# ntnu-yjyjames/nano-vectordb

Measured on AMD Instinct MI355X. Metric: QPS + effective HBM GB/s, flat-scan top-10 d=768, higher is better.
Workload: dtype f16

## Files before the change

nano-vectordb_amd/csrc/kernels_exact.h:

```cpp
#pragma once
#include <hip/hip_runtime.h>

#include "nvdb_common.h"

namespace nvdbhip {

struct Cand { float score; uint32_t row; };

constexpr int DT_F32 = 1, DT_F16 = 2, DT_I8 = 3;
constexpr float NEG_INF = -__builtin_huge_valf();

__device__ __forceinline__ bool better(float s1, uint32_t i1, float s2, uint32_t i2) {
  return (s1 > s2) || (s1 == s2 && i1 < i2);
}
__device__ __forceinline__ float half_bits_to_float(uint32_t h16) {
  return static_cast<float>(__builtin_bit_cast(_Float16, static_cast<unsigned short>(h16)));
}
__device__ __forceinline__ float readlane_f(float v, int l) {
  return __builtin_bit_cast(float, __builtin_amdgcn_readlane(__builtin_bit_cast(int, v), l));
}
__device__ __forceinline__ uint32_t readlane_u(uint32_t v, int l) {
  return static_cast<uint32_t>(__builtin_amdgcn_readlane(static_cast<int>(v), l));
}
__device__ __forceinline__ float hsum8(const float (&a)[8]) {
// ... 200 lines not shown
  if (wave != 0) return;
#pragma unroll
  for (int g = 0; g < QG; ++g) {
    for (int w = 1; w < 4; ++w) {
      const uint32_t c = lds_cnt[w][g];
      for (uint32_t j = 0; j < c; ++j) {
        const float cs = lds_s[w][g][j];
        const uint32_t cid = lds_id[w][g][j];
        if (wtk_accepts(tk[g], k, cs, cid)) wtk_insert(tk[g], k, cs, cid, lane);
      }
    }
    const uint32_t qi = qbase + g;
    const bool own = qi >= qg0 && qi < nq;
    if (own && tk[g].cnt > 0) {
      uint32_t slot0 = 0;
      if (lane == 0) slot0 = atomicAdd(&cnt[qi], tk[g].cnt);
      slot0 = readlane_u(slot0, 0);
      if (static_cast<uint32_t>(lane) < tk[g].cnt) {
        const uint32_t slot = slot0 + lane;
        if (slot < cap) cand[static_cast<uint64_t>(qi) * cap + slot] = Cand{tk[g].s, tk[g].id};
        else overflow[qi] = 1u;
      }
    }
  }
}

__device__ __forceinline__ void fold_sticky_words(uint32_t* any_overflow) {
  const uint32_t viol = __hip_atomic_load(any_overflow - 6, __ATOMIC_RELAXED, __HIP_MEMORY_SCOPE_AGENT);
  const uint32_t logovf = __hip_atomic_load(any_overflow - 5, __ATOMIC_RELAXED, __HIP_MEMORY_SCOPE_AGENT);
  if (viol) atomicAdd(any_overflow + 7, viol);
  if (logovf) atomicOr(any_overflow + 8, 1u);
}

__device__ __forceinline__ void select_body(
    const uint32_t q, const uint32_t tid, const uint32_t nth, Cand* e,
    Cand* __restrict__ cand, uint32_t* __restrict__ cnt, uint32_t cap, uint32_t k, const float* __restrict__ slack,
    float* __restrict__ thr, uint32_t* __restrict__ overflow, int mode, uint64_t row_base,
    unsigned long long* __restrict__ out_ids, float* __restrict__ out_scores, uint32_t out_k, uint32_t* __restrict__ any_overflow,
    float* __restrict__ xcdw, bool fold_sticky) {
  __shared__ uint32_t s_keep;
  if (xcdw != nullptr && q == 0 && tid == 0) {
    float sp[8], mean = 0.f;
    bool all = true;
#pragma unroll
    for (int x = 0; x < 8; ++x) {
      const float us = xcdw[8 + x], tiles = xcdw[16 + x];
      all = all && us > 0.f && tiles > 0.f;
      sp[x] = tiles / fmaxf(us, 1e-3f);
      mean += sp[x] * 0.125f;
    }
    if (all) {
      float w[8], wsum = 0.f;
#pragma unroll
      for (int x = 0; x < 8; ++x) {
        w[x] = fminf(fmaxf(0.5f * xcdw[x] + 0.5f * sp[x] / mean, 0.9f), 1.1f);
        wsum += w[x];
      }
#pragma unroll
      for (int x = 0; x < 8; ++x) xcdw[x] = w[x] * (8.f / wsum);
    }
#pragma unroll
    for (int x = 8; x < 24; ++x) xcdw[x] = 0.f;
  }
  uint32_t m = (mode == 2) ? out_k : cnt[q];
  if (m > cap) { if (tid == 0) overflow[q] = 1u; m = cap; }
  if ((mode & 1) && tid == 0) {
    if (overflow[q]) { atomicOr(any_overflow, 1u); if (mode == 1) atomicOr(any_overflow + 6, 1u); }
    if (mode == 1 && fold_sticky) fold_sticky_words(any_overflow);
  }
  Cand* mine = cand + static_cast<uint64_t>(q) * cap;
  if (m <= 512) {
    __shared__ float s_kth;
    if (tid == 0) { s_keep = 0; s_kth = NEG_INF; }
    for (uint32_t i = tid; i < m; i += nth) e[i] = mine[i];
    __syncthreads();
    Cand my[2];
    uint32_t rk[2] = {0xFFFFFFFFu, 0xFFFFFFFFu};
#pragma unroll
    for (int u = 0; u < 2; ++u) {
      const uint32_t i = tid + u * nth;
      if (i < m) {
        my[u] = e[i];
        uint32_t r = 0;
        uint32_t j = 0;
        for (; j + 8 <= m; j += 8) {
          Cand o[8];
#pragma unroll
          for (int v = 0; v < 8; ++v) o[v] = e[j + v];
#pragma unroll
          for (int v = 0; v < 8; ++v) r += better(o[v].score, o[v].row, my[u].score, my[u].row) ? 1u : 0u;
        }
        for (; j < m; ++j) { const Cand o = e[j]; r += better(o.score, o.row, my[u].score, my[u].row) ? 1u : 0u; }
        rk[u] = r;
        if (r == k - 1) s_kth = my[u].score;
      }
    }
    __syncthreads();
    if (mode & 1) {
      const uint32_t c = m < k ? m : k;
#pragma unroll
      for (int u = 0; u < 2; ++u)
        if (rk[u] < c) { out_ids[static_cast<uint64_t>(q) * out_k + rk[u]] = row_base + my[u].row; out_scores[static_cast<uint64_t>(q) * out_k + rk[u]] = my[u].score; }
      for (uint32_t j = c + tid; j < out_k; j += nth) { out_ids[static_cast<uint64_t>(q) * out_k + j] = ~0ull; out_scores[static_cast<uint64_t>(q) * out_k + j] = NEG_INF; }
      return;
    }
    const float sl = slack ? slack[q] : 0.f;
    const float t = fmaxf(s_kth - sl, thr[q]);
    uint32_t local = 0;
#pragma unroll
    for (int u = 0; u < 2; ++u) if (rk[u] != 0xFFFFFFFFu) local += (sl > 0.f ? (my[u].score >= t) : (rk[u] < k)) ? 1u : 0u;
    if (local) atomicAdd(&s_keep, local);
    __syncthreads();
    const uint32_t keep = s_keep;
#pragma unroll
    for (int u = 0; u < 2; ++u) if (rk[u] < keep) mine[rk[u]] = my[u];
    if (tid == 0) { cnt[q] = (mode == 2) ? 0u : keep; thr[q] = t; }
    return;
  }
  uint32_t M2 = 1;
  while (M2 < m) M2 <<= 1;
  for (uint32_t i = tid; i < M2; i += nth) e[i] = (i < m) ? mine[i] : Cand{NEG_INF, 0xFFFFFFFFu};
  __syncthreads();
  for (uint32_t size = 2; size <= M2; size <<= 1) {
    for (uint32_t stride = size >> 1; stride > 0; stride >>= 1) {
      for (uint32_t i = tid; i < (M2 >> 1); i += nth) {
        const uint32_t a = 2 * i - (i & (stride - 1));
        const uint32_t b = a + stride;
        const bool desc = ((a & size) == 0);
        const Cand ea = e[a], eb = e[b];
        const bool b_better = better(eb.score, eb.row, ea.score, ea.row);
        if (b_better == desc) { e[a] = eb; e[b] = ea; }
      }
      __syncthreads();
    }
  }
  if (mode & 1) {
    const uint32_t c = m < k ? m : k;
    for (uint32_t j = tid; j < out_k; j += nth) {
      const bool have = j < c;
      out_ids[static_cast<uint64_t>(q) * out_k + j] = have ? (row_base + e[j].row) : ~0ull;
      out_scores[static_cast<uint64_t>(q) * out_k + j] = have ? e[j].score : NEG_INF;
    }
    return;
  }
  const float kth = (m >= k) ? e[k - 1].score : NEG_INF;
  const float sl = slack ? slack[q] : 0.f;
  const float t = fmaxf(kth - sl, thr[q]);
  if (tid == 0) s_keep = 0;
  __syncthreads();
  uint32_t local = 0;
  if (sl > 0.f) { for (uint32_t i = tid; i < m; i += nth) local += (e[i].score >= t) ? 1u : 0u; }
  else { for (uint32_t i = tid; i < m; i += nth) local += (i < k) ? 1u : 0u; }
  if (local) atomicAdd(&s_keep, local);
  __syncthreads();
  const uint32_t keep = s_keep;
  for (uint32_t i = tid; i < keep; i += nth) mine[i] = e[i];
  if (tid == 0) { cnt[q] = (mode == 2) ? 0u : keep; thr[q] = t; }
}

static __global__ __launch_bounds__(256) void select_kernel(
    Cand* __restrict__ cand, uint32_t* __restrict__ cnt, uint32_t cap, uint32_t k, const float* __restrict__ slack,
    float* __restrict__ thr, uint32_t* __restrict__ overflow, int mode, uint64_t row_base,
    unsigned long long* __restrict__ out_ids, float* __restrict__ out_scores, uint32_t out_k, uint32_t* __restrict__ any_overflow,
    float* __restrict__ xcdw) {
  extern __shared__ __attribute__((aligned(16))) char smem_raw[];
  select_body(blockIdx.x, threadIdx.x, blockDim.x, reinterpret_cast<Cand*>(smem_raw), cand, cnt, cap, k, slack, thr, overflow, mode, row_base,
              out_ids, out_scores, out_k, any_overflow, xcdw, blockIdx.x == 0);
}

static __global__ __launch_bounds__(256) void init_search_kernel(uint32_t* __restrict__ cnt, uint32_t* __restrict__ overflow,
                                                          float* __restrict__ thr, uint32_t* __restrict__ misc, uint32_t nq_pad,
                                                          uint32_t* __restrict__ prog, uint32_t prog_words) {
  const uint32_t i = blockIdx.x * 256 + threadIdx.x;
  if (i < nq_pad) { cnt[i] = 0; overflow[i] = 0; thr[i] = NEG_INF; }
  if (i < 8) misc[i] = 0;
  for (uint32_t j = i; j < prog_words; j += gridDim.x * 256) prog[j] = 0xFFFFFFFFu;
}

template <int DT, bool ALIGNED>
__global__ __launch_bounds__(256) void rescore_kernel(
    const void* __restrict__ rows, const float* __restrict__ scales, uint32_t dim, const float* __restrict__ q32,
    Cand* __restrict__ cand, const uint32_t* __restrict__ cnt, uint32_t cap, const float* __restrict__ ebound,
    uint32_t* __restrict__ violations, unsigned long long* __restrict__ total_cands) {
  const uint32_t q = blockIdx.x;
  uint32_t m = cnt[q];
  if (m > cap) m = cap;
  if (m == 0) return;
  extern __shared__ __attribute__((aligned(16))) char smem_raw[];
  float* qptr = reinterpret_cast<float*>(smem_raw);
  const uint32_t qstride = (dim + 3u) & ~3u;
  for (uint32_t j = threadIdx.x; j < qstride; j += 256) qptr[j] = (j < dim) ? q32[static_cast<uint64_t>(q) * dim + j] : 0.f;
  __syncthreads();
  const float eb = ebound ? ebound[q] : 0.f;
  Cand* mine = cand + static_cast<uint64_t>(q) * cap;
  for (uint32_t i = threadIdx.x; i < m; i += 256) {
    const Cand c = mine[i];
    float sc[1];
    const float scale = (DT == DT_I8) ? scales[c.row] : 1.f;
    exact_scores<DT, 1, ALIGNED>(row_ptr<DT>(rows, c.row, dim), qptr, qstride, dim, scale, sc);
    if (ebound && eb >= 0.f && !(__builtin_fabsf(sc[0] - c.score) <= eb)) atomicAdd(violations, 1u);
// ... 50 lines not shown

struct FinalSelect {
  int mode;
  uint32_t k, out_k;
  uint64_t row_base;
  unsigned long long* out_ids;
  float* out_scores;
  float* thr;
  uint32_t* overflow;
  uint32_t* any_overflow;
  uint32_t* ticket;
  uint32_t* status_out;
};

template <int DT>
__global__ __launch_bounds__(256) void rescore_lds_kernel(
    const void* __restrict__ rows, const float* __restrict__ scales, uint32_t dim, const float* __restrict__ q32,
    Cand* __restrict__ cand, uint32_t* __restrict__ cnt, uint32_t cap, const float* __restrict__ ebound,
    uint32_t* __restrict__ violations, unsigned long long* __restrict__ total_cands, uint32_t cpp, FinalSelect fs) {
  constexpr uint32_t BPE = (DT == DT_F32) ? 4 : (DT == DT_F16 ? 2 : 1);
  const uint32_t q = blockIdx.x, tid = threadIdx.x;
  uint32_t m = cnt[q];
  if (m > cap) m = cap;
  if (m == 0 && fs.mode == 0) return;
  extern __shared__ __attribute__((aligned(16))) char smem_raw[];
  const uint32_t qstride = (dim + 3u) & ~3u, row_bytes = dim * BPE, slot_bytes = row_bytes + 16, cpr = row_bytes >> 4;
  float* qptr = reinterpret_cast<float*>(smem_raw);
  char* slots = smem_raw + qstride * 4;
  __shared__ Cand s_cand[32];
  for (uint32_t j = tid; j < dim; j += 256) qptr[j] = q32[static_cast<uint64_t>(q) * dim + j];
  const float eb = ebound ? ebound[q] : 0.f;
  Cand* mine = cand + static_cast<uint64_t>(q) * cap;
  const uint32_t j8 = tid & 7u, grp = tid >> 3;
  const uint32_t body = (DT == DT_I8) ? (dim & ~15u) : (dim & ~7u);
  for (uint32_t base = 0; base < m; base += cpp) {
    const uint32_t nrows = (m - base < cpp) ? m - base : cpp;
    __syncthreads();
    if (tid < nrows) s_cand[tid] = mine[base + tid];
    __syncthreads();
    for (uint32_t c = tid; c < nrows * cpr; c += 256) {
      const uint32_t r = c / cpr, ch = c - r * cpr;
      const uint4 v = *reinterpret_cast<const uint4*>(static_cast<const char*>(rows) + static_cast<uint64_t>(s_cand[r].row) * row_bytes + ch * 16);
      *reinterpret_cast<uint4*>(slots + r * slot_bytes + ch * 16) = v;
    }
    __syncthreads();
    if (grp < nrows) {
      const Cand c = s_cand[grp];
      const void* rp = slots + grp * slot_bytes;
      float acc = 0.f;
      uint32_t e = j8;
#pragma unroll 8
      for (; e < body; e += 8) acc = __builtin_fmaf(qptr[e], load1<DT>(rp, e), acc);
      float s = acc + __shfl_xor(acc, 4);
      s = s + __shfl_xor(s, 1);
      s = s + __shfl_xor(s, 2);
      uint32_t t = body;
      if (t < dim) {
        if constexpr (DT == DT_F32) {
          if (dim - t >= 4) {
            for (int u = 0; u < 4; ++u) { const float p = qptr[t + u] * load1<DT>(rp, t + u); s = s + p; }
            t += 4;
          }
        }
        for (; t < dim; ++t) s = __builtin_fmaf(qptr[t], load1<DT>(rp, t), s);
      }
      if constexpr (DT == DT_I8) s = s * scales[c.row];
      if (j8 == 0) {
        if (ebound && eb >= 0.f && !(__builtin_fabsf(s - c.score) <= eb)) atomicAdd(violations, 1u);
        mine[base + grp].score = s;
      }
    }
  }
  if (fs.mode == 0) return;
  __syncthreads();
  select_body(q, tid, 256u, reinterpret_cast<Cand*>(smem_raw), cand, cnt, cap, fs.k, nullptr, fs.thr, fs.overflow, fs.mode, fs.row_base,
              fs.out_ids, fs.out_scores, fs.out_k, fs.any_overflow, nullptr, false);
  if (fs.ticket == nullptr) return;
  asm volatile("s_waitcnt vmcnt(0)" ::: "memory");
  __syncthreads();
  if (tid == 0) {
    const uint32_t t = __hip_atomic_fetch_add(fs.ticket, 1u, __ATOMIC_RELAXED, __HIP_MEMORY_SCOPE_AGENT);
    if (t == gridDim.x - 1) {
      if (fs.mode == 1) fold_sticky_words(fs.any_overflow);
      if (fs.status_out != nullptr) {
#pragma unroll
        for (int i = 0; i < 8; ++i) fs.status_out[i] = __hip_atomic_load(fs.any_overflow - 6 + i, __ATOMIC_RELAXED, __HIP_MEMORY_SCOPE_AGENT);
      }
    }
  }
}

static __global__ __launch_bounds__(256) void merge_topk_kernel(
    const unsigned long long* __restrict__ ids, const float* __restrict__ scores, uint32_t nshards, uint32_t nq,
    uint32_t k, unsigned long long* __restrict__ out_ids, float* __restrict__ out_scores, size_t stride_ids_bytes,
    size_t stride_scores_bytes) {
  extern __shared__ __attribute__((aligned(16))) char smem_raw[];
  const uint32_t m = nshards * k, q = blockIdx.x;
  float* s = reinterpret_cast<float*>(smem_raw);
  unsigned long long* id = reinterpret_cast<unsigned long long*>(smem_raw + ((m * 4 + 15) & ~15u));
  for (uint32_t i = threadIdx.x; i < m; i += 256) {
    const uint32_t sh = i / k, j = i % k;
    s[i] = reinterpret_cast<const float*>(reinterpret_cast<const char*>(scores) + sh * stride_scores_bytes)[static_cast<uint64_t>(q) * k + j];
    id[i] = reinterpret_cast<const unsigned long long*>(reinterpret_cast<const char*>(ids) + sh * stride_ids_bytes)[static_cast<uint64_t>(q) * k + j];
  }
  __syncthreads();
  for (uint32_t i = threadIdx.x; i < m; i += 256) {
    const float si = s[i];
    const unsigned long long ii = id[i];
    uint32_t rank = 0;
// ... 41 lines not shown
```

nano-vectordb_amd/csrc/nvdb_corpus.cpp:

```cpp
#include "nvdb_ctx.h"
#include "kernels_corpus.h"

namespace {

std::string g_create_err;

void free_corpus(nvdb_hip_ctx* c) {
  if (c->owned) {
    if (c->rows) (void)hipFree(c->rows);
    if (c->scales) (void)hipFree(c->scales);
  }
  if (c->shadow16) { (void)hipFree(c->shadow16); c->shadow16 = nullptr; }
  if (c->shadow8) { (void)hipFree(c->shadow8); c->shadow8 = nullptr; }
  if (c->shadow8_scales) { (void)hipFree(c->shadow8_scales); c->shadow8_scales = nullptr; }
  c->rows = nullptr; c->scales = nullptr; c->owned = false; c->n = 0; c->dim = 0; c->fdim = 0; c->dtype = 0; c->max_norm = 0.f;
  c->cap_hint = 0;
  c->q8shadow = false; c->resid_max = 0.f; c->filter_max_norm = 0.f;
  c->shadow_demoted = false; c->last_filter_kind = 0;
  c->range_valid = false; c->range_total = 0;
  parts_drop(c);
  c->nmasks = 0;
}

nvdb_status compute_max_norm(nvdb_hip_ctx* c) {
// ... 340 lines not shown
  if (k == "path") { if (value < 0 || value > 2) return fail(c, NVDB_ERR_INVALID, "path must be 0,1,2"); c->opt_path = value; }
  else if (k == "chunk0_rows") { if (value < 256) return fail(c, NVDB_ERR_INVALID, "chunk0_rows must be >= 256"); c->opt_chunk0 = value; }
  else if (k == "cand_cap") { if (value < 0 || value > SELECT_MAX_CAP) return fail(c, NVDB_ERR_INVALID, "cand_cap out of range"); c->opt_cap = value; }
  else if (k == "time_kernels") { c->opt_time_kernels = value ? 1 : 0; }
  else if (k == "sync_every") { if (value < 1 || (value & (value - 1))) return fail(c, NVDB_ERR_INVALID, "sync_every must be a power of two"); c->opt_sync_every = value; }
  else if (k == "sync_lead") { if (value < 1) return fail(c, NVDB_ERR_INVALID, "sync_lead must be >= 1"); c->opt_sync_lead = value; }
  else if (k == "sibling_sync") { c->opt_sibling_sync = value ? 1 : 0; }
  else if (k == "f32_shadow") { c->opt_f32_shadow = value ? 1 : 0; }
  else if (k == "q8_shadow") { c->opt_q8_shadow = value < 0 ? -1 : value ? 1 : 0; }
  else if (k == "q8_auto_min_rows") { if (value < 1) return fail(c, NVDB_ERR_INVALID, "q8_auto_min_rows must be >= 1"); c->opt_q8_auto_min_rows = value; }
  else if (k == "q8_auto_max_mb") { if (value < 0 || value > (int64_t(1) << 30)) return fail(c, NVDB_ERR_INVALID, "q8_auto_max_mb out of range"); c->opt_q8_auto_max_mb = value; }
#ifdef NVDB_HIP_DEV
  else if (k == "mfma16") { c->opt_mfma16 = value ? 1 : 0; }
  else if (k == "i8_wide") { c->opt_i8_wide = value ? 1 : 0; }
  else if (k == "i8_pipe") { c->opt_i8_pipe = value ? 1 : 0; }
  else if (k == "i8_waves8") { c->opt_i8_waves8 = value ? 1 : 0; }
  else if (k == "i8_mfma16") { c->opt_i8_mfma16 = value ? 1 : 0; }
  else if (k == "i8_small8") { c->opt_i8_small8 = value ? 1 : 0; }
#else
  else if (k == "mfma16" || k == "i8_wide" || k == "i8_pipe" || k == "i8_mfma16" || k == "i8_small8") { if (!value) return fail(c, NVDB_ERR_UNSUPPORTED, k + " = 0 selects a developer-build kernel variant (libnvdb_hip_dev.so)"); }
  else if (k == "i8_waves8") { if (value) return fail(c, NVDB_ERR_UNSUPPORTED, "i8_waves8 = 1 selects a developer-build kernel variant (libnvdb_hip_dev.so)"); }
#endif

  else if (k == "i8_defer") { c->opt_i8_defer = value ? 1 : 0; }
  else if (k == "xcd_balance") { c->opt_xcd_balance = value ? 1 : 0; }
  else if (k == "i8_lo_bits") { if (value < 2 || value > 7) return fail(c, NVDB_ERR_INVALID, "i8_lo_bits must be in [2,7]"); c->opt_i8_lo_bits = value; }
  else if (k == "boot_tiles") { if (value < 0 || value > SELECT_MAX_CAP) return fail(c, NVDB_ERR_INVALID, "boot_tiles out of range"); c->opt_boot_tiles = value; }
#ifdef NVDB_HIP_DEV
  else if (k == "debug_rows") { c->dbg_rows = value < 0 ? 0 : value; }
#endif
  else if (k == "waves8") { c->opt_waves8 = value ? 1 : 0; }
  else if (k == "fuse") { c->opt_fuse = value ? 1 : 0; }
  else if (k == "zero_copy") { c->opt_zero_copy = value ? 1 : 0; }
  else if (k == "exact_mfma") { c->opt_exact_mfma = value ? 1 : 0; }
  else if (k == "exact_img") { c->opt_exact_img = value ? 1 : 0; }
  else if (k == "exact_prescan") { c->opt_exact_prescan = value ? 1 : 0; }
  else if (k == "exact_wgs") { if (value < 1 || value > 16) return fail(c, NVDB_ERR_INVALID, "exact_wgs must be in [1,16]"); c->opt_exact_wgs = value; }
  else if (k == "exact_lds") { if (value < 0 || value > 2) return fail(c, NVDB_ERR_INVALID, "exact_lds must be 0, 1 or 2"); c->opt_exact_lds = value; }
  else if (k == "time_launches") { c->opt_time_launches = value ? 1 : 0; }
  else if (k == "tile_permute") { c->opt_tile_permute = value ? 1 : 0; }
  else if (k == "rescore8") { c->opt_rescore8 = value < 0 ? 0 : (value > 2 ? 2 : value); }
  else if (k == "mfma_boot") { c->opt_mfma_boot = value ? 1 : 0; }
  else if (k == "refine_v2") { c->opt_refine_v2 = value < 0 ? 0 : (value > 2 ? 2 : value); }
  else if (k == "refine_pinned") { c->opt_refine_pinned = value ? 1 : 0; }
  else if (k == "refine_dbg_q") { if (value < 0) return fail(c, NVDB_ERR_INVALID, "refine_dbg_q must be >= 0"); c->opt_refine_dbg_q = value; }
  else if (k == "largek_budget_mb") { if (value < 1) return fail(c, NVDB_ERR_INVALID, "largek_budget_mb must be >= 1"); c->opt_largek_budget_mb = value; }
  else if (k == "range_max_mb") { if (value < 1) return fail(c, NVDB_ERR_INVALID, "range_max_mb must be >= 1"); c->opt_range_max_mb = value; }
  else if (k == "chunk_growth") { if (value != 0 && (value < 2 || value > 64)) return fail(c, NVDB_ERR_INVALID, "chunk_growth must be 0 (automatic) or in [2,64]"); c->opt_growth = value; }
  else if (k == "min_filter_batch") { if (value < 1) return fail(c, NVDB_ERR_INVALID, "min_filter_batch must be >= 1"); c->opt_min_filter_batch = value; }
  else return fail(c, NVDB_ERR_INVALID, "unknown option: " + k);
  return NVDB_OK;
}

nvdb_status nvdb_hip_shadow_info(const nvdb_hip_ctx* c, uint64_t* out4) {
  if (!c || !out4) return NVDB_ERR_INVALID;
  out4[0] = c->q8shadow ? 1u : 0u;
  out4[1] = c->q8shadow ? q8_shadow_bytes(c->n, c->dim) : 0u;
  out4[2] = c->shadow_demoted ? 1u : 0u;
  out4[3] = c->last_filter_kind;
  return NVDB_OK;
}

nvdb_status nvdb_hip_get_stats(nvdb_hip_ctx* c, nvdb_hip_scan_stats* stats) {
  if (!c || !stats) return NVDB_ERR_INVALID;
  if (c->stats_lazy) {
    c->stats_lazy = false;
// ... 38 lines not shown
```

nano-vectordb_amd/csrc/nvdb_ctx.h:

```cpp
#pragma once
#pragma GCC visibility push(default)
#include "../../include/nvdb_hip.h"
#ifdef NVDB_HIP_DEV
#include "../../include/nvdb_hip_dev.h"
#endif
#pragma GCC visibility pop

#include <hip/hip_runtime.h>
#include <hip/hip_ext.h>

#include <algorithm>
#include <atomic>
#include <chrono>
#include <cmath>
#include <cstdio>
#include <cstdlib>
#include <cstring>
#include <set>
#include <string>
#include <thread>
#include <type_traits>
#include <vector>

#include "kernels_exact.h"
// ... 49 lines not shown
  int64_t opt_q8_auto_max_mb = 16384;
  float* shadow8_scales = nullptr;
  _Float16* shadow16 = nullptr;
  uint32_t fdim = 0;
  DevBuf qdelta;
  int64_t opt_i8_wide = 1;
  int64_t opt_i8_waves8 = 0;
  int64_t opt_i8_defer = 0;
  int64_t opt_i8_mfma16 = 1;
  int64_t opt_i8_pipe = 1;
  int64_t opt_waves8 = 1;
  void* pinned = nullptr;
  void* pinned_dev = nullptr;
  size_t pinned_bytes = 0;
  bool perm_on = false;
  int64_t opt_tile_permute = 1;
  uint32_t cap_hint = 0;
  bool stats_lazy = false;
  hipEvent_t launch_e0 = nullptr, launch_e1 = nullptr;
  std::vector<hipEvent_t> kl_pool;
  uint32_t prog_slot = 0;
  int64_t opt_time_launches = 0;
  int64_t opt_exact_lds = 1;
  int64_t opt_exact_img = 1;
  int64_t opt_exact_wgs = 1;
  int64_t opt_exact_prescan = 1;
  int64_t opt_exact_mfma = 1;
  int64_t opt_rescore8 = 2;

  DevBuf q32, q16, qscale, qinv, ebound, slack, thr, cnt, overflow, cand, out_ids, out_scores, misc, hitlog, prog;
  DevBuf hostblock;
  DevBuf tickets;
  int64_t opt_fuse = 1;
  int64_t opt_zero_copy = 1;
  bool status_by_kernel = false;
  size_t q32_dirty = 0;
  DevBuf rq, rcand, rout_ids, rout_dist;
  DevBuf rdbg;
  DevBuf xcdw;
  int64_t opt_xcd_balance = 1;
  int64_t opt_i8_lo_bits = 7;
  int64_t opt_boot_tiles = 0;
  int64_t opt_i8_small8 = 1;
  int64_t dbg_rows = 0;
  DevBuf lk_scores, lk_sel, lk_hist, lk_state;
  int64_t opt_refine_pinned = 0;
  int64_t opt_refine_dbg_q = 0;
  void* rpinned = nullptr;
  size_t rpinned_bytes = 0;
  int64_t opt_largek_budget_mb = 8192;
  DevBuf rg_radius, rg_kept, rg_off, rg_idx, rg_q, rg_desc, rg_taken, rg_slab;
  DevBuf rg_pcnt, rg_maskof;
  DevBuf rg_ids, rg_scores;
  uint64_t range_total = 0;
  bool range_valid = false;
  int64_t opt_range_max_mb = 4096;

  int64_t opt_path = 0, opt_chunk0 = 512, opt_cap = 0, opt_min_filter_batch = 1, opt_growth = 0;

  nvdb_hip_scan_stats stats{};
  uint32_t last_nq = 0, last_cap = 0;
  bool last_filter = false;
  std::vector<hipEvent_t> ev_pool;
  std::vector<std::pair<int, int>> ev_filter;
  struct KLaunch { hipEvent_t e0, e1; double flops, bytes; };
  std::vector<KLaunch> klaunch;
// ... 86 lines not shown

inline bool i8_two_stage(const nvdb_hip_ctx* c) { return filter_is_i8(c) && c->opt_i8_wide; }

inline uint32_t filter_nb(const nvdb_hip_ctx* c, uint32_t nq) {
  if (filter_is_i8(c) && (!i8_two_stage(c) || c->fdim > 768)) return 1u;
  if (!filter_is_i8(c) && c->fdim > 768) return 1u;
  return nq <= 128 ? 1u : 2u;
}

inline bool corpus_padded(const nvdb_hip_ctx* c) { return c->owned || c->shadow16 != nullptr || (c->shadow8 != nullptr && filter_is_i8(c)); }
inline bool f16_m16_build(const nvdb_hip_ctx* c, uint32_t nb) { return nb == 2 && c->opt_mfma16; }
constexpr uint32_t f16_m16_tile_rows(uint32_t dim) { return dim <= 384 ? 64u : 32u; }
constexpr uint32_t i8w_tile_rows(uint32_t dim) { return dim <= 768 ? I8W_TILE_ROWS : FILTER_ROWS; }
inline uint32_t filter_tile_rows(const nvdb_hip_ctx* c, uint32_t nq) {
  if (filter_is_i8(c)) return i8_two_stage(c) ? i8w_tile_rows(c->fdim) : FILTER_ROWS;
  return (c->fdim <= 768 && f16_m16_build(c, filter_nb(c, nq))) ? f16_m16_tile_rows(c->fdim) : FILTER_ROWS;
}
constexpr uint32_t f16_filter_qpb(uint32_t dim, uint32_t nb) { return dim > 1536 ? 64u : dim > 768 ? 128u : 128u * nb; }
constexpr uint32_t f16_m16_qpb(uint32_t nqb, uint32_t wpb) { return 16u * nqb * wpb; }
inline uint32_t filter_qpb(const nvdb_hip_ctx* c, uint32_t nq) { return filter_is_i8(c) ? 128u * filter_nb(c, nq) : f16_filter_qpb(c->fdim, filter_nb(c, nq)); }
inline bool i8_pipelined(const nvdb_hip_ctx* c, uint32_t nb) { return nb == 2 && c->opt_i8_pipe; }
inline bool i8_stage2_in_loop(const nvdb_hip_ctx* c) { return c->opt_i8_defer != 0 || c->i8_scales_signed; }
inline bool i8_logs_survivors(const nvdb_hip_ctx* c, uint32_t nb) { return i8_pipelined(c, nb) && !i8_stage2_in_loop(c); }

inline hipEvent_t get_event(nvdb_hip_ctx* c, size_t idx) {
  while (c->ev_pool.size() <= idx) { hipEvent_t e; (void)hipEventCreate(&e); c->ev_pool.push_back(e); }
  return c->ev_pool[idx];
}

nvdb_status launch_init_search(nvdb_hip_ctx* c, hipStream_t s, uint32_t nq_pad, uint32_t prog_words);
nvdb_status launch_scan_exact(nvdb_hip_ctx* c, hipStream_t s, uint32_t row_lo, uint32_t row_hi, const float* q32, uint32_t nq, uint32_t k,
                              const float* thr, uint32_t cap, uint32_t reserve);
nvdb_status launch_select(nvdb_hip_ctx* c, hipStream_t s, uint32_t nq, uint32_t cap, uint32_t k, const float* slack, int mode, uint64_t* out_ids,
                          float* out_scores, uint32_t out_k);
nvdb_status launch_rescore(nvdb_hip_ctx* c, hipStream_t s, const float* q32, uint32_t nq, uint32_t cap, FinalSelect fs = FinalSelect{}, bool* fused = nullptr);
nvdb_status search_largek(nvdb_hip_ctx* c, hipStream_t s, const float* dev_q, uint32_t nq, uint32_t k, uint64_t* dev_out_ids, float* dev_out_scores,
                          uint32_t n_rows = 0, Cand* seed_cand = nullptr, uint32_t* seed_cnt = nullptr, uint32_t seed_cap = 0);
nvdb_status score_matrix_batch(nvdb_hip_ctx* c, uint32_t nq, size_t per_query_bytes, size_t held_bytes, uint32_t& QB, uint32_t& QG);
nvdb_status launch_score_matrix(nvdb_hip_ctx* c, hipStream_t s, const float* q32, uint32_t nq, float* scores, uint64_t ld, uint32_t n, uint32_t QG, bool mfma_ok);
nvdb_status launch_sort_keys(nvdb_hip_ctx* c, hipStream_t s, unsigned long long* keys, uint32_t K2, uint32_t lists);
nvdb_status launch_prep_q16(nvdb_hip_ctx* c, hipStream_t s, const float* dev_q, uint32_t nq, uint32_t nq_pad, const PrepInit& pinit);
nvdb_status launch_prep_q8(nvdb_hip_ctx* c, hipStream_t s, const float* dev_q, uint32_t nq, uint32_t nq_pad, const PrepInit& pinit);
nvdb_status launch_filter_f16(nvdb_hip_ctx* c, hipStream_t s, uint32_t row_lo, uint32_t row_hi, uint32_t nq, uint32_t QT, uint32_t cap);
nvdb_status launch_filter_i8(nvdb_hip_ctx* c, hipStream_t s, uint32_t row_lo, uint32_t row_hi, uint32_t nq, uint32_t QT, uint32_t cap);
nvdb_status launch_boot_f16(nvdb_hip_ctx* c, hipStream_t s, uint32_t n0, uint32_t nq, uint32_t QT, uint32_t cap, uint32_t nb);
nvdb_status launch_boot_i8(nvdb_hip_ctx* c, hipStream_t s, uint32_t n0, uint32_t nq, uint32_t QT, uint32_t cap);
nvdb_status corpus_alloc_padded(nvdb_hip_ctx* c, uint64_t n, uint32_t dim, uint32_t dtype, void** rows, float** scales);
nvdb_status corpus_take_ownership(nvdb_hip_ctx* c, void* dev_rows, float* dev_scales, uint64_t n, uint32_t dim, uint32_t dtype, uint64_t global_row_base);
void parts_drop(nvdb_hip_ctx* c);
void parts_destroy(nvdb_hip_ctx* c);
nvdb_status ensure_q32(nvdb_hip_ctx* c, hipStream_t s, size_t qbytes);
nvdb_status zero_q32_pad(nvdb_hip_ctx* c, hipStream_t s, size_t qbytes);
nvdb_status next_prog_region(nvdb_hip_ctx* c, hipStream_t s, uint32_t nwg, uint32_t** out);
ScatterArgs scatter_args(nvdb_hip_ctx* c, uint32_t cap, uint32_t trows = 0);
float filter_events_ms(const nvdb_hip_ctx* c);
nvdb_status sum_candidates(nvdb_hip_ctx* c, unsigned long long* total);

inline nvdb_status raise_lds_limit(nvdb_hip_ctx* c, const void* fn, size_t bytes) {
  if (c->lds_attr_set.count(fn)) return NVDB_OK;
  HIPCHK(c, hipFuncSetAttribute(fn, hipFuncAttributeMaxDynamicSharedMemorySize, static_cast<int>(bytes)));
  c->lds_attr_set.insert(fn);
  return NVDB_OK;
}

inline uint32_t filter_grid(const nvdb_hip_ctx* c, uint32_t QT) {
  const uint32_t nwg = (static_cast<uint32_t>(c->num_cu) / QT) * QT;
  return nwg ? nwg : QT;
// ... 54 lines not shown
```

nano-vectordb_amd/csrc/nvdb_launch_exact.cpp:

```cpp
#include "nvdb_ctx.h"
#include "kernels_exact_mfma.h"
#include "kernels_largek.h"

namespace nvdbhip {

nvdb_status launch_init_search(nvdb_hip_ctx* c, hipStream_t s, uint32_t nq_pad, uint32_t prog_words) {
  init_search_kernel<<<(nq_pad + 255) / 256, 256, 0, s>>>(static_cast<uint32_t*>(c->cnt.p), static_cast<uint32_t*>(c->overflow.p),
                                                          static_cast<float*>(c->thr.p), static_cast<uint32_t*>(c->misc.p), nq_pad,
                                                          static_cast<uint32_t*>(c->prog.p), prog_words);
  HIPCHK(c, hipGetLastError());
  return NVDB_OK;
}


template <int QG>
nvdb_status launch_scan_exact_qg(nvdb_hip_ctx* c, hipStream_t s, uint32_t row_lo, uint32_t row_hi, const float* q32,
                                 uint32_t nq, uint32_t k, const float* thr, uint32_t P, uint32_t cap) {
  const dim3 grid(P, (nq + QG - 1) / QG);
  Cand* cand = static_cast<Cand*>(c->cand.p);
  uint32_t* cnt = static_cast<uint32_t*>(c->cnt.p);
  uint32_t* ovf = static_cast<uint32_t*>(c->overflow.p);
  const bool al = aligned_rows(c->dtype, c->dim);
  const uint32_t qstride = (c->dim + 3u) & ~3u;
  const size_t lds = static_cast<size_t>(QG) * qstride * 4 + static_cast<size_t>(4) * QG * 64 * 8 + 4 * QG * 4;
// ... 75 lines not shown
    default: NVDB_SCAN_MFMA(128); break;
  }
#undef NVDB_SCAN_MFMA
  HIPCHK(c, hipGetLastError());
  return NVDB_OK;
}

nvdb_status launch_scan_exact(nvdb_hip_ctx* c, hipStream_t s, uint32_t row_lo, uint32_t row_hi, const float* q32,
                              uint32_t nq, uint32_t k, const float* thr, uint32_t cap, uint32_t reserve) {
  if (k > WAVE_KMAX) return fail(c, NVDB_ERR_INTERNAL, "scan_exact: k beyond the wavefront-resident lists (64)");
  if (c->opt_exact_mfma && nq > 8 && exact_mfma_dim(c->dim) && row_hi - row_lo >= 64u * EXACT_MFMA_ROWS) {
    if (c->dtype == NVDB_DTYPE_F32) return launch_scan_exact_mfma<DT_F32>(c, s, row_lo, row_hi, q32, nq, k, thr, cap, reserve);
    if (c->dtype == NVDB_DTYPE_F16) return launch_scan_exact_mfma<DT_F16>(c, s, row_lo, row_hi, q32, nq, k, thr, cap, reserve);
    return launch_scan_exact_mfma<DT_I8>(c, s, row_lo, row_hi, q32, nq, k, thr, cap, reserve);
  }
  uint32_t QG = nq >= 8 ? 8 : (nq >= 4 ? 4 : (nq >= 2 ? 2 : 1));
  while (QG > 1 && static_cast<size_t>(QG) * (((c->dim + 3u) & ~3u) * 4 + 4 * 64 * 8 + 16) > 60 * 1024) QG >>= 1;
  if (static_cast<size_t>((c->dim + 3u) & ~3u) * 4 + 4 * 64 * 8 + 16 > 60 * 1024) return fail(c, NVDB_ERR_UNSUPPORTED, "dim too large for the exact kernel's LDS query staging (max ~14800)");
  const uint32_t gy = (nq + QG - 1) / QG;
  const uint32_t rows = row_hi - row_lo;
  uint32_t pmax = (cap > reserve + k) ? (cap - reserve) / k : 1;
  uint32_t P = std::max<uint32_t>(1, (8u * static_cast<uint32_t>(c->num_cu) + gy - 1) / gy);
  P = std::min(P, std::max<uint32_t>(1, (rows + 255) / 256));
  P = std::max<uint32_t>(1, std::min(P, pmax));
  switch (QG) {
    case 8: return launch_scan_exact_qg<8>(c, s, row_lo, row_hi, q32, nq, k, thr, P, cap);
    case 4: return launch_scan_exact_qg<4>(c, s, row_lo, row_hi, q32, nq, k, thr, P, cap);
    case 2: return launch_scan_exact_qg<2>(c, s, row_lo, row_hi, q32, nq, k, thr, P, cap);
    default: return launch_scan_exact_qg<1>(c, s, row_lo, row_hi, q32, nq, k, thr, P, cap);
  }
}

nvdb_status launch_select(nvdb_hip_ctx* c, hipStream_t s, uint32_t nq, uint32_t cap, uint32_t k, const float* slack,
                          int mode, uint64_t* out_ids, float* out_scores, uint32_t out_k) {
  const void* fn = reinterpret_cast<const void*>(select_kernel);
  if (nvdb_status ls = raise_lds_limit(c, fn, SELECT_MAX_CAP * sizeof(Cand))) return ls;
  uint32_t cap2 = 1;
  while (cap2 < cap) cap2 <<= 1;
  static_assert(SELECT_MAX_CAP * sizeof(Cand) <= 64 * 1024 && (SELECT_MAX_CAP & (SELECT_MAX_CAP - 1)) == 0, "select_kernel LDS");
  select_kernel<<<nq, 256, cap2 * sizeof(Cand), s>>>(static_cast<Cand*>(c->cand.p), static_cast<uint32_t*>(c->cnt.p), cap, k, slack,
                                                   static_cast<float*>(c->thr.p), static_cast<uint32_t*>(c->overflow.p), mode,
                                                   c->row_base, reinterpret_cast<unsigned long long*>(out_ids), out_scores, out_k,
                                                   static_cast<uint32_t*>(c->misc.p) + 6,
                                                   c->opt_xcd_balance ? static_cast<float*>(c->xcdw.p) : nullptr);
  HIPCHK(c, hipGetLastError());
  return NVDB_OK;
}

nvdb_status launch_rescore(nvdb_hip_ctx* c, hipStream_t s, const float* q32, uint32_t nq, uint32_t cap, FinalSelect fs, bool* fused) {
  Cand* cand = static_cast<Cand*>(c->cand.p);
  uint32_t* cnt = static_cast<uint32_t*>(c->cnt.p);
  if (fused) *fused = false;
  const float* eb = static_cast<const float*>(c->ebound.p);
  uint32_t* viol = static_cast<uint32_t*>(c->misc.p);
  unsigned long long* tot = reinterpret_cast<unsigned long long*>(static_cast<char*>(c->misc.p) + 8);
  const size_t rs_lds = static_cast<size_t>((c->dim + 3u) & ~3u) * 4;
  const size_t row_bytes = static_cast<size_t>(c->dim) * bpe_of(c->dtype);
  uint32_t cpp = 32;
  while (cpp > 1 && rs_lds + cpp * (row_bytes + 16) > 60 * 1024) cpp >>= 1;
  if (c->opt_rescore8 >= 2 && (row_bytes & 15) == 0 && cpp >= 4) {
    size_t lds = rs_lds + cpp * (row_bytes + 16);
    if (fs.mode != 0) {
      uint32_t cap2 = 1;
      while (cap2 < cap) cap2 <<= 1;
      lds = std::max(lds, cap2 * sizeof(Cand));
    }
    const void* fn = c->dtype == NVDB_DTYPE_F32 ? reinterpret_cast<const void*>(rescore_lds_kernel<DT_F32>)
                   : c->dtype == NVDB_DTYPE_F16 ? reinterpret_cast<const void*>(rescore_lds_kernel<DT_F16>) : reinterpret_cast<const void*>(rescore_lds_kernel<DT_I8>);
    if (lds > 48 * 1024)
      if (nvdb_status ls = raise_lds_limit(c, fn, SELECT_MAX_CAP * sizeof(Cand))) return ls;
    if (c->dtype == NVDB_DTYPE_F32) rescore_lds_kernel<DT_F32><<<nq, 256, lds, s>>>(c->rows, c->scales, c->dim, q32, cand, cnt, cap, eb, viol, tot, cpp, fs);
    else if (c->dtype == NVDB_DTYPE_F16) rescore_lds_kernel<DT_F16><<<nq, 256, lds, s>>>(c->rows, c->scales, c->dim, q32, cand, cnt, cap, eb, viol, tot, cpp, fs);
    else rescore_lds_kernel<DT_I8><<<nq, 256, lds, s>>>(c->rows, c->scales, c->dim, q32, cand, cnt, cap, eb, viol, tot, cpp, fs);
    HIPCHK(c, hipGetLastError());
    if (fused) *fused = fs.mode != 0;
    return NVDB_OK;
  }
// ... 227 lines not shown
```

nano-vectordb_amd/csrc/nvdb_search.cpp:

```cpp
#include "nvdb_plan.h"

namespace nvdbhip {

nvdb_status ensure_hostblock(nvdb_hip_ctx* c, size_t out_bytes) {
  const size_t need = 64 + out_bytes;
  if (c->hostblock.p && c->hostblock.bytes >= need) return NVDB_OK;
  HIPCHK(c, hipDeviceSynchronize());
  void* np = nullptr;
  const size_t want = std::max<size_t>(need + need / 2, static_cast<size_t>(1) << 20);
  HIPCHK(c, hipMalloc(&np, want));
  if (c->misc.p) HIPCHK(c, hipMemcpy(np, c->misc.p, 64, hipMemcpyDeviceToDevice));
  else HIPCHK(c, hipMemset(np, 0, 64));
  if (c->hostblock.p) HIPCHK(c, hipFree(c->hostblock.p));
  else if (c->misc.p) HIPCHK(c, hipFree(c->misc.p));
  c->hostblock.p = np; c->hostblock.bytes = want;
  c->misc.p = np; c->misc.bytes = 64;
  return NVDB_OK;
}

nvdb_status ensure_q32(nvdb_hip_ctx* c, hipStream_t s, size_t qbytes) {
  const size_t before = c->q32.p ? c->q32.bytes : 0;
  if (nvdb_status st = ensure(c, c->q32, qbytes + 8 * static_cast<size_t>(c->dim) * 4)) return st;
  if (c->q32.bytes != before) { HIPCHK(c, hipMemsetAsync(c->q32.p, 0, c->q32.bytes, s)); c->q32_dirty = 0; }
  return NVDB_OK;
// ... 53 lines not shown
  for (const auto& w : workspace)
    if ((p.prep || !w.filter_flow) && (st = ensure(c, w.buf, w.bytes))) return st;
  c->stats = nvdb_hip_scan_stats{};
  c->stats.path = p.route;
  c->last_nq = nq; c->last_cap = cap; c->last_filter = p.route == ROUTE_FILTER;
  c->ev_filter.clear();
  c->prog_slot = 0;
  if (p.route == ROUTE_FILTER) c->perm_on = p.perm_on;
  c->last_filter_kind = p.route != ROUTE_FILTER ? 0u : p.shadow ? 2u : c->dtype == NVDB_DTYPE_I8 ? 3u : 1u;

  if (host_q && !p.prep_inits) { HIPCHK(c, hipMemcpyAsync(const_cast<float*>(dev_q), host_q, static_cast<size_t>(nq) * c->dim * 4, hipMemcpyDefault, s)); host_q = nullptr; }
  if (!p.prep_inits && (st = launch_init_search(c, s, p.nq_pad, QT > 1 ? p.prog_words : 0u))) return st;
  const PrepInit pinit = p.prep_inits ? PrepInit{static_cast<uint32_t*>(c->cnt.p), static_cast<float*>(c->thr.p), static_cast<uint32_t*>(c->misc.p),
                                                 static_cast<uint32_t*>(c->prog.p), QT > 1 ? p.prog_words : 0u, static_cast<uint32_t*>(c->tickets.p), host_q, const_cast<float*>(dev_q)}
                                      : PrepInit{nullptr, nullptr, nullptr, nullptr, 0u, nullptr, nullptr, nullptr};
  if (p.prep && (st = filter_is_i8(c) ? launch_prep_q8(c, s, dev_q, nq, p.nq_pad, pinit) : launch_prep_q16(c, s, dev_q, nq, p.nq_pad, pinit))) return st;
  const float* thr = static_cast<const float*>(c->thr.p);
  const float* slack = static_cast<const float*>(c->slack.p);

  if (p.route == ROUTE_ANYK) return search_largek(c, s, dev_q, nq, k, dev_out_ids, dev_out_scores);
  if (p.route == ROUTE_EXACT) {
    if (p.head && (st = launch_scan_exact(c, s, 0, p.head, dev_q, nq, k_eff, nullptr, cap, 0))) return st;
    if (p.head && (st = launch_select(c, s, nq, cap, k_eff, nullptr, 0, nullptr, nullptr, 0))) return st;
    if ((st = launch_scan_exact(c, s, p.head, n, dev_q, nq, k_eff, p.head ? thr : nullptr, cap, p.head ? k_eff : 0))) return st;
    c->stats.chunks = p.head ? 2 : 1;
    c->stats.rows_scanned = c->n;
    return launch_select(c, s, nq, cap, k_eff, nullptr, final_mode, dev_out_ids, dev_out_scores, k);
  }

  if (p.boot == BOOT_MFMA) st = launch_boot(c, s, p.boot_rows, nq, QT, cap, filter_nb(c, nq));
  else if (p.boot == BOOT_ANYK_SEEDED) st = search_largek(c, s, dev_q, nq, k_eff, nullptr, nullptr, p.r0, static_cast<Cand*>(c->cand.p), static_cast<uint32_t*>(c->cnt.p), cap);
  else st = launch_scan_exact(c, s, 0, p.r0, dev_q, nq, k_eff, nullptr, cap, 0);
  if (st) return st;
  if ((st = launch_select(c, s, nq, cap, k_eff, slack, p.boot == BOOT_MFMA ? 2 : 0, nullptr, nullptr, p.boot == BOOT_MFMA ? p.boot_tiles : 0))) return st;
  size_t ev = 0;
  for (uint32_t r = p.r0; r < p.n_al;) {
    const uint32_t hi = chunk_end(p, r);
    nvdb_hip_ctx::KLaunch kl{nullptr, nullptr, 0.0, 0.0};
    const bool acct = c->opt_time_kernels && c->klaunch.size() < 8192;
    if (acct) {
      for (hipEvent_t* e : {&kl.e0, &kl.e1}) {
        if (!c->kl_pool.empty()) { *e = c->kl_pool.back(); c->kl_pool.pop_back(); }
        else HIPCHK(c, hipEventCreate(e));
      }
      kl.flops = 2.0 * nq * static_cast<double>(std::min(hi, n) - r) * c->dim;
      kl.bytes = static_cast<double>(std::min(hi, n) - r) * (filter_is_i8(c) ? c->fdim + 4.0 : c->fdim * 2.0);
      c->launch_e0 = kl.e0; c->launch_e1 = kl.e1;
    } else if (time_filter) {
      c->launch_e0 = get_event(c, ev); c->launch_e1 = get_event(c, ev + 1);
    }
    if (time_filter && acct) { HIPCHK(c, hipEventRecord(get_event(c, ev), s)); }
    st = launch_filter(c, s, r, hi, nq, QT, cap);
    c->launch_e0 = nullptr; c->launch_e1 = nullptr;
    if (st) return st;
    if (time_filter && acct) { HIPCHK(c, hipEventRecord(get_event(c, ev + 1), s)); }
    if (time_filter) { c->ev_filter.emplace_back(ev, ev + 1); ev += 2; }
    if (acct) c->klaunch.push_back(kl);
    if ((st = launch_select(c, s, nq, cap, k_eff, slack, 0, nullptr, nullptr, 0))) return st;
    c->stats.chunks++;
    c->stats.rows_scanned += static_cast<uint64_t>(hi - r) * QT;
    r = hi;
  }
  if (p.tail_exact && (st = launch_scan_exact(c, s, p.n_al, n, dev_q, nq, std::min(k_eff, WAVE_KMAX), thr, cap, 0))) return st;
  if (p.tail_exact) c->stats.rows_scanned += static_cast<uint64_t>(n - p.n_al) * QT;
  FinalSelect fs{};
  if (c->opt_fuse)
    fs = FinalSelect{final_mode, k_eff, k, c->row_base, reinterpret_cast<unsigned long long*>(dev_out_ids), dev_out_scores, static_cast<float*>(c->thr.p),
                     static_cast<uint32_t*>(c->overflow.p), static_cast<uint32_t*>(c->misc.p) + 6,
                     p.prep_inits ? static_cast<uint32_t*>(c->tickets.p) + (FUSE_TICKETS - 1) : nullptr, p.prep_inits ? status_out : nullptr};
  if (fs.mode == 1 && fs.ticket == nullptr) fs.mode = 0;
  bool fused = false;
  if ((st = launch_rescore(c, s, dev_q, nq, cap, fs, &fused))) return st;
  if (fused) { c->status_by_kernel = fs.status_out != nullptr; return NVDB_OK; }
  return launch_select(c, s, nq, cap, k_eff, nullptr, final_mode, dev_out_ids, dev_out_scores, k);
}

float filter_events_ms(const nvdb_hip_ctx* c) {
  float total = 0.f;
  for (auto& pr : c->ev_filter) { float ms = 0.f; if (hipEventElapsedTime(&ms, c->ev_pool[pr.first], c->ev_pool[pr.second]) == hipSuccess) total += ms; }
  return total;
}

nvdb_status sum_candidates(nvdb_hip_ctx* c, unsigned long long* total) {
  *total = 0;
  if (!c->last_nq) return NVDB_OK;
  std::vector<uint32_t> cn(c->last_nq);
  HIPCHK(c, hipMemcpy(cn.data(), c->cnt.p, c->last_nq * 4, hipMemcpyDeviceToHost));
  for (uint32_t v : cn) *total += std::min(v, c->last_cap);
  return NVDB_OK;
}

// ... 250 lines not shown
```

Measured before the change: 148,400.

## Tighten select threshold by exact-rescoring top-2k candidates in shadow mode

In the shadow (approximate filter) path, the select kernel now rescans the top 2k candidates at full precision against the f32 query. It takes the exact k-th score minus the error bound as the pruning threshold, replacing the approximate k-th minus slack. A tighter threshold should keep fewer candidates per chunk and cut the cost of later filter and rescore passes. The price is extra row reads, a per-query copy of the query into LDS, and an O(M^2) rank step inside every select launch.

```diff
diff --git a/nano-vectordb_amd/csrc/kernels_exact.h b/nano-vectordb_amd/csrc/kernels_exact.h
--- a/nano-vectordb_amd/csrc/kernels_exact.h
+++ b/nano-vectordb_amd/csrc/kernels_exact.h
@@ -256,13 +256,76 @@
   if (logovf) atomicOr(any_overflow + 8, 1u);
 }
 
+template <int DT>
+__device__ __forceinline__ float score8(const void* rp, const float* qptr, uint32_t dim, uint32_t j8) {
+  const uint32_t body = (DT == DT_I8) ? (dim & ~15u) : (dim & ~7u);
+  float acc = 0.f;
+#pragma unroll 8
+  for (uint32_t e = 0; e < body; e += 8) acc = __builtin_fmaf(qptr[e + j8], load1<DT>(rp, e + j8), acc);
+  float s = acc + __shfl_xor(acc, 4);
+  s = s + __shfl_xor(s, 1);
+  s = s + __shfl_xor(s, 2);
+  uint32_t t = body;
+  if (t < dim) {
+    if constexpr (DT == DT_F32) {
+      if (dim - t >= 4) {
+        for (int u = 0; u < 4; ++u) { const float p = qptr[t + u] * load1<DT>(rp, t + u); s = s + p; }
+        t += 4;
+      }
+    }
+    for (; t < dim; ++t) s = __builtin_fmaf(qptr[t], load1<DT>(rp, t), s);
+  }
+  return s;
+}
+
+struct ExactBar {
+  const void* rows;
+  const float* q32;
+  const float* ebound;
+  uint32_t dim, n_rows;
+  uint32_t q_off;
+};
+constexpr uint32_t EXACT_BAR_MAX = 2 * 64;
+
+template <int XDT>
+__device__ __forceinline__ float exact_kth(const ExactBar& xb, uint32_t q, float* qptr, const uint32_t* s_row, float* s_sc, float* s_B,
+                                           uint32_t M, uint32_t k, uint32_t tid, uint32_t nth) {
+  for (uint32_t j = tid; j < xb.dim; j += nth) qptr[j] = xb.q32[static_cast<uint64_t>(q) * xb.dim + j];
+  if (tid == 0) *s_B = NEG_INF;
+  __syncthreads();
+  const uint32_t j8 = tid & 7u, grp = tid >> 3, per = nth >> 3;
+  for (uint32_t base = 0; base < M; base += per) {
+    const uint32_t i = base + grp;
+    if (i >= M) continue;
+    const uint32_t row = s_row[i];
+    float s = NEG_INF;
+    if (row < xb.n_rows) s = score8<XDT>(row_ptr<XDT>(xb.rows, row, xb.dim), qptr, xb.dim, j8);
+    if (j8 == 0) s_sc[i] = (s == s) ? s : NEG_INF;
+  }
+  __syncthreads();
+  for (uint32_t i = tid; i < M; i += nth) {
+    const float si = s_sc[i];
+    uint32_t r = 0;
+    for (uint32_t j = 0; j < M; ++j) { const float sj = s_sc[j]; r += (sj > si || (sj == si && j < i)) ? 1u : 0u; }
+    if (r == k - 1) *s_B = si;
+  }
+  __syncthreads();
+  return *s_B;
+}
+
+template <int XDT>
 __device__ __forceinline__ void select_body(
     const uint32_t q, const uint32_t tid, const uint32_t nth, Cand* e,
     Cand* __restrict__ cand, uint32_t* __restrict__ cnt, uint32_t cap, uint32_t k, const float* __restrict__ slack,
     float* __restrict__ thr, uint32_t* __restrict__ overflow, int mode, uint64_t row_base,
     unsigned long long* __restrict__ out_ids, float* __restrict__ out_scores, uint32_t out_k, uint32_t* __restrict__ any_overflow,
-    float* __restrict__ xcdw, bool fold_sticky) {
+    float* __restrict__ xcdw, bool fold_sticky, const ExactBar& xb_in) {
+  ExactBar xb = xb_in;
+  if constexpr (XDT != 0) asm volatile("" : "+v"(xb.rows), "+v"(xb.q32), "+v"(xb.ebound), "+v"(xb.n_rows), "+v"(xb.q_off));
   __shared__ uint32_t s_keep;
+  __shared__ uint32_t s_xrow[XDT != 0 ? EXACT_BAR_MAX : 1];
+  __shared__ float s_xsc[XDT != 0 ? EXACT_BAR_MAX : 1], s_xB;
+  float* xq = reinterpret_cast<float*>(reinterpret_cast<char*>(e) + (XDT != 0 ? xb.q_off : 0u));
   if (xcdw != nullptr && q == 0 && tid == 0) {
     float sp[8], mean = 0.f;
     bool all = true;
@@ -329,7 +392,17 @@
       return;
     }
     const float sl = slack ? slack[q] : 0.f;
-    const float t = fmaxf(s_kth - sl, thr[q]);
+    float bar = s_kth - sl;
+    if constexpr (XDT != 0) {
+      const float xeb = m >= k ? xb.ebound[q] : -1.f;
+      if (xeb >= 0.f) {
+        const uint32_t M = m < 2 * k ? m : 2 * k;
+#pragma unroll
+        for (int u = 0; u < 2; ++u) if (rk[u] < M) s_xrow[rk[u]] = my[u].row;
+        bar = exact_kth<XDT>(xb, q, xq, s_xrow, s_xsc, &s_xB, M, k, tid, nth) - xeb;
+      }
+    }
+    const float t = fmaxf(bar, thr[q]);
     uint32_t local = 0;
 #pragma unroll
     for (int u = 0; u < 2; ++u) if (rk[u] != 0xFFFFFFFFu) local += (sl > 0.f ? (my[u].score >= t) : (rk[u] < k)) ? 1u : 0u;
@@ -369,7 +442,16 @@
   }
   const float kth = (m >= k) ? e[k - 1].score : NEG_INF;
   const float sl = slack ? slack[q] : 0.f;
-  const float t = fmaxf(kth - sl, thr[q]);
+  float bar = kth - sl;
+  if constexpr (XDT != 0) {
+    const float xeb = m >= k ? xb.ebound[q] : -1.f;
+    if (xeb >= 0.f) {
+      const uint32_t M = m < 2 * k ? m : 2 * k;
+      for (uint32_t i = tid; i < M; i += nth) s_xrow[i] = e[i].row;
+      bar = exact_kth<XDT>(xb, q, xq, s_xrow, s_xsc, &s_xB, M, k, tid, nth) - xeb;
+    }
+  }
+  const float t = fmaxf(bar, thr[q]);
   if (tid == 0) s_keep = 0;
   __syncthreads();
   uint32_t local = 0;
@@ -382,14 +464,15 @@
   if (tid == 0) { cnt[q] = (mode == 2) ? 0u : keep; thr[q] = t; }
 }
 
-static __global__ __launch_bounds__(256) void select_kernel(
+template <int XDT>
+__global__ __launch_bounds__(256) void select_kernel(
     Cand* __restrict__ cand, uint32_t* __restrict__ cnt, uint32_t cap, uint32_t k, const float* __restrict__ slack,
     float* __restrict__ thr, uint32_t* __restrict__ overflow, int mode, uint64_t row_base,
     unsigned long long* __restrict__ out_ids, float* __restrict__ out_scores, uint32_t out_k, uint32_t* __restrict__ any_overflow,
-    float* __restrict__ xcdw) {
+    float* __restrict__ xcdw, ExactBar xb) {
   extern __shared__ __attribute__((aligned(16))) char smem_raw[];
-  select_body(blockIdx.x, threadIdx.x, blockDim.x, reinterpret_cast<Cand*>(smem_raw), cand, cnt, cap, k, slack, thr, overflow, mode, row_base,
-              out_ids, out_scores, out_k, any_overflow, xcdw, blockIdx.x == 0);
+  select_body<XDT>(blockIdx.x, threadIdx.x, blockDim.x, reinterpret_cast<Cand*>(smem_raw), cand, cnt, cap, k, slack, thr, overflow, mode, row_base,
+              out_ids, out_scores, out_k, any_overflow, xcdw, blockIdx.x == 0, xb);
 }
 
 static __global__ __launch_bounds__(256) void init_search_kernel(uint32_t* __restrict__ cnt, uint32_t* __restrict__ overflow,
@@ -506,7 +589,6 @@
   const float eb = ebound ? ebound[q] : 0.f;
   Cand* mine = cand + static_cast<uint64_t>(q) * cap;
   const uint32_t j8 = tid & 7u, grp = tid >> 3;
-  const uint32_t body = (DT == DT_I8) ? (dim & ~15u) : (dim & ~7u);
   for (uint32_t base = 0; base < m; base += cpp) {
     const uint32_t nrows = (m - base < cpp) ? m - base : cpp;
     __syncthreads();
@@ -520,24 +602,7 @@
     __syncthreads();
     if (grp < nrows) {
       const Cand c = s_cand[grp];
-      const void* rp = slots + grp * slot_bytes;
-      float acc = 0.f;
-      uint32_t e = j8;
-#pragma unroll 8
-      for (; e < body; e += 8) acc = __builtin_fmaf(qptr[e], load1<DT>(rp, e), acc);
-      float s = acc + __shfl_xor(acc, 4);
-      s = s + __shfl_xor(s, 1);
-      s = s + __shfl_xor(s, 2);
-      uint32_t t = body;
-      if (t < dim) {
-        if constexpr (DT == DT_F32) {
-          if (dim - t >= 4) {
-            for (int u = 0; u < 4; ++u) { const float p = qptr[t + u] * load1<DT>(rp, t + u); s = s + p; }
-            t += 4;
-          }
-        }
-        for (; t < dim; ++t) s = __builtin_fmaf(qptr[t], load1<DT>(rp, t), s);
-      }
+      float s = score8<DT>(slots + grp * slot_bytes, qptr, dim, j8);
       if constexpr (DT == DT_I8) s = s * scales[c.row];
       if (j8 == 0) {
         if (ebound && eb >= 0.f && !(__builtin_fabsf(s - c.score) <= eb)) atomicAdd(violations, 1u);
@@ -547,8 +612,8 @@
   }
   if (fs.mode == 0) return;
   __syncthreads();
-  select_body(q, tid, 256u, reinterpret_cast<Cand*>(smem_raw), cand, cnt, cap, fs.k, nullptr, fs.thr, fs.overflow, fs.mode, fs.row_base,
-              fs.out_ids, fs.out_scores, fs.out_k, fs.any_overflow, nullptr, false);
+  select_body<0>(q, tid, 256u, reinterpret_cast<Cand*>(smem_raw), cand, cnt, cap, fs.k, nullptr, fs.thr, fs.overflow, fs.mode, fs.row_base,
+              fs.out_ids, fs.out_scores, fs.out_k, fs.any_overflow, nullptr, false, ExactBar{});
   if (fs.ticket == nullptr) return;
   asm volatile("s_waitcnt vmcnt(0)" ::: "memory");
   __syncthreads();
diff --git a/nano-vectordb_amd/csrc/nvdb_corpus.cpp b/nano-vectordb_amd/csrc/nvdb_corpus.cpp
--- a/nano-vectordb_amd/csrc/nvdb_corpus.cpp
+++ b/nano-vectordb_amd/csrc/nvdb_corpus.cpp
@@ -396,6 +396,7 @@
   else if (k == "waves8") { c->opt_waves8 = value ? 1 : 0; }
   else if (k == "fuse") { c->opt_fuse = value ? 1 : 0; }
   else if (k == "zero_copy") { c->opt_zero_copy = value ? 1 : 0; }
+  else if (k == "shadow_exact_thr") { c->opt_shadow_exact_thr = value ? 1 : 0; }
   else if (k == "exact_mfma") { c->opt_exact_mfma = value ? 1 : 0; }
   else if (k == "exact_img") { c->opt_exact_img = value ? 1 : 0; }
   else if (k == "exact_prescan") { c->opt_exact_prescan = value ? 1 : 0; }
diff --git a/nano-vectordb_amd/csrc/nvdb_ctx.h b/nano-vectordb_amd/csrc/nvdb_ctx.h
--- a/nano-vectordb_amd/csrc/nvdb_ctx.h
+++ b/nano-vectordb_amd/csrc/nvdb_ctx.h
@@ -105,6 +105,7 @@
   DevBuf hostblock;
   DevBuf tickets;
   int64_t opt_fuse = 1;
+  int64_t opt_shadow_exact_thr = 1;
   int64_t opt_zero_copy = 1;
   bool status_by_kernel = false;
   size_t q32_dirty = 0;
@@ -257,7 +258,7 @@
 nvdb_status launch_scan_exact(nvdb_hip_ctx* c, hipStream_t s, uint32_t row_lo, uint32_t row_hi, const float* q32, uint32_t nq, uint32_t k,
                               const float* thr, uint32_t cap, uint32_t reserve);
 nvdb_status launch_select(nvdb_hip_ctx* c, hipStream_t s, uint32_t nq, uint32_t cap, uint32_t k, const float* slack, int mode, uint64_t* out_ids,
-                          float* out_scores, uint32_t out_k);
+                          float* out_scores, uint32_t out_k, const float* q32 = nullptr);
 nvdb_status launch_rescore(nvdb_hip_ctx* c, hipStream_t s, const float* q32, uint32_t nq, uint32_t cap, FinalSelect fs = FinalSelect{}, bool* fused = nullptr);
 nvdb_status search_largek(nvdb_hip_ctx* c, hipStream_t s, const float* dev_q, uint32_t nq, uint32_t k, uint64_t* dev_out_ids, float* dev_out_scores,
                           uint32_t n_rows = 0, Cand* seed_cand = nullptr, uint32_t* seed_cnt = nullptr, uint32_t seed_cap = 0);
diff --git a/nano-vectordb_amd/csrc/nvdb_launch_exact.cpp b/nano-vectordb_amd/csrc/nvdb_launch_exact.cpp
--- a/nano-vectordb_amd/csrc/nvdb_launch_exact.cpp
+++ b/nano-vectordb_amd/csrc/nvdb_launch_exact.cpp
@@ -131,17 +131,23 @@
 }
 
 nvdb_status launch_select(nvdb_hip_ctx* c, hipStream_t s, uint32_t nq, uint32_t cap, uint32_t k, const float* slack,
-                          int mode, uint64_t* out_ids, float* out_scores, uint32_t out_k) {
-  const void* fn = reinterpret_cast<const void*>(select_kernel);
-  if (nvdb_status ls = raise_lds_limit(c, fn, SELECT_MAX_CAP * sizeof(Cand))) return ls;
+                          int mode, uint64_t* out_ids, float* out_scores, uint32_t out_k, const float* q32) {
+  constexpr size_t XQ_MAX = 16 * 1024;
   uint32_t cap2 = 1;
   while (cap2 < cap) cap2 <<= 1;
   static_assert(SELECT_MAX_CAP * sizeof(Cand) <= 64 * 1024 && (SELECT_MAX_CAP & (SELECT_MAX_CAP - 1)) == 0, "select_kernel LDS");
-  select_kernel<<<nq, 256, cap2 * sizeof(Cand), s>>>(static_cast<Cand*>(c->cand.p), static_cast<uint32_t*>(c->cnt.p), cap, k, slack,
+  const size_t qbytes = static_cast<size_t>(c->dim) * 4;
+  const bool f16 = c->dtype == NVDB_DTYPE_F16;
+  if (q32 != nullptr && ((mode & 1) || k > WAVE_KMAX || qbytes > XQ_MAX || (!f16 && c->dtype != NVDB_DTYPE_F32)))
+    return fail(c, NVDB_ERR_INTERNAL, "select: exact bar asked for a list it does not serve");
+  auto kern = q32 == nullptr ? select_kernel<0> : f16 ? select_kernel<DT_F16> : select_kernel<DT_F32>;
+  if (nvdb_status ls = raise_lds_limit(c, reinterpret_cast<const void*>(kern), SELECT_MAX_CAP * sizeof(Cand) + (q32 ? XQ_MAX : 0))) return ls;
+  const ExactBar xb{c->rows, q32, static_cast<const float*>(c->ebound.p), c->dim, static_cast<uint32_t>(c->n), static_cast<uint32_t>(cap2 * sizeof(Cand))};
+  kern<<<nq, 256, cap2 * sizeof(Cand) + (q32 ? qbytes : 0), s>>>(static_cast<Cand*>(c->cand.p), static_cast<uint32_t*>(c->cnt.p), cap, k, slack,
                                                    static_cast<float*>(c->thr.p), static_cast<uint32_t*>(c->overflow.p), mode,
                                                    c->row_base, reinterpret_cast<unsigned long long*>(out_ids), out_scores, out_k,
                                                    static_cast<uint32_t*>(c->misc.p) + 6,
-                                                   c->opt_xcd_balance ? static_cast<float*>(c->xcdw.p) : nullptr);
+                                                   c->opt_xcd_balance ? static_cast<float*>(c->xcdw.p) : nullptr, xb);
   HIPCHK(c, hipGetLastError());
   return NVDB_OK;
 }
diff --git a/nano-vectordb_amd/csrc/nvdb_search.cpp b/nano-vectordb_amd/csrc/nvdb_search.cpp
--- a/nano-vectordb_amd/csrc/nvdb_search.cpp
+++ b/nano-vectordb_amd/csrc/nvdb_search.cpp
@@ -109,7 +109,8 @@
   else if (p.boot == BOOT_ANYK_SEEDED) st = search_largek(c, s, dev_q, nq, k_eff, nullptr, nullptr, p.r0, static_cast<Cand*>(c->cand.p), static_cast<uint32_t*>(c->cnt.p), cap);
   else st = launch_scan_exact(c, s, 0, p.r0, dev_q, nq, k_eff, nullptr, cap, 0);
   if (st) return st;
-  if ((st = launch_select(c, s, nq, cap, k_eff, slack, p.boot == BOOT_MFMA ? 2 : 0, nullptr, nullptr, p.boot == BOOT_MFMA ? p.boot_tiles : 0))) return st;
+  const float* xthr_q = (p.shadow && k_eff <= WAVE_KMAX && c->opt_shadow_exact_thr) ? dev_q : nullptr;
+  if ((st = launch_select(c, s, nq, cap, k_eff, slack, p.boot == BOOT_MFMA ? 2 : 0, nullptr, nullptr, p.boot == BOOT_MFMA ? p.boot_tiles : 0, xthr_q))) return st;
   size_t ev = 0;
   for (uint32_t r = p.r0; r < p.n_al;) {
     const uint32_t hi = chunk_end(p, r);
@@ -133,7 +134,7 @@
     if (time_filter && acct) { HIPCHK(c, hipEventRecord(get_event(c, ev + 1), s)); }
     if (time_filter) { c->ev_filter.emplace_back(ev, ev + 1); ev += 2; }
     if (acct) c->klaunch.push_back(kl);
-    if ((st = launch_select(c, s, nq, cap, k_eff, slack, 0, nullptr, nullptr, 0))) return st;
+    if ((st = launch_select(c, s, nq, cap, k_eff, slack, 0, nullptr, nullptr, 0, xthr_q))) return st;
     c->stats.chunks++;
     c->stats.rows_scanned += static_cast<uint64_t>(hi - r) * QT;
     r = hi;
```

Result: faster. 161,700, median of 6 (+9.0%).
